# dyollb/segmantic

Measured on AMD Instinct MI355X. Metric: 3D UNet train voxels/s on 128^3 bf16, higher is better.
Workload: dtype bf16

## Files before the change

### include/segmi.h

```cpp
#ifndef SEGMI_H_
#define SEGMI_H_

#include <stddef.h>
#include <stdint.h>

#ifdef __cplusplus
extern "C" {
#endif

#define SEGMI_VERSION 1

enum { SEGMI_F32 = 0, SEGMI_BF16 = 1, SEGMI_F16 = 2 };
enum { SEGMI_OK = 0, SEGMI_EINVAL = -1, SEGMI_EUNSUPPORTED = -2, SEGMI_ELAUNCH = -3,
       SEGMI_EDATA = -4  };

typedef struct segmi_act {
  void* data;
  int32_t n, d, h, w;
  int32_t c;
  int32_t ld;
} segmi_act;

int segmi_version(void);
const char* segmi_last_error(void);
// ... 113 lines not shown
int segmi_bn_eval_affine(int c, const float* gamma, const float* beta,
                         const float* running_mean, const float* running_var, float eps,
                         float* scale, float* shift, void* stream);
int segmi_bn_act_fwd(int dtype, const segmi_act* x, const segmi_act* y, const float* scale,
                     const float* shift, const float* prelu_alpha, const segmi_act* residual,
                     float dropout_p, uint32_t dropout_seed, void* stream);
int segmi_bn_act_bwd_rows(const segmi_act* x);
int segmi_bn_act_bwd_reduce(int dtype, const segmi_act* dy, const segmi_act* x,
                            const float* mean, const float* invstd, const float* gamma,
                            const float* beta, const float* prelu_alpha, float* red_partials,
                            float dropout_p, uint32_t dropout_seed,
                            const segmi_bn_bwd_fin* fin , void* stream);
int segmi_bn_act_bwd_finalize(const float* red_partials, int rows, int c, double count,
                              const float* gamma, const float* invstd, float* dgamma,
                              float* dbeta, float* dalpha, float* coef, void* stream);
int segmi_bn_act_bwd_fused_ok(int dtype, const segmi_act* dy, const segmi_act* x, const segmi_act* dx);
int segmi_bn_act_bwd_fused_rows(const segmi_act* x);
int segmi_bn_act_bwd_fused_wgs(int dtype, const segmi_act* x, int max_wgs);
int segmi_bn_act_bwd_fused(int dtype, const segmi_act* dy, const segmi_act* x, const segmi_act* dx,
                           const float* mean, const float* invstd, const float* gamma, const float* beta,
                           const float* prelu_alpha, float* red_partials, const segmi_bn_bwd_fin* fin,
                           int max_wgs, void* stream);
unsigned segmi_fused_timeouts(int reset);
int segmi_fused_test_hook(unsigned poll_limit, int no_publish);
int segmi_bn_act_bwd_apply(int dtype, const segmi_act* dy, const segmi_act* x,
                           const segmi_act* dx, const float* mean, const float* invstd,
                           const float* gamma, const float* beta, const float* prelu_alpha,
                           const float* coef, float dropout_p, uint32_t dropout_seed, void* stream);
int segmi_bn_act_bwd_apply_conv_ok(int dtype, const segmi_act* dy, const segmi_act* x, const segmi_act* dx,
                                   const segmi_act* out);
int segmi_bn_act_bwd_apply_conv(int dtype, const segmi_act* dy, const segmi_act* x, const segmi_act* dx,
                                const float* mean, const float* invstd, const float* gamma, const float* beta,
                                const float* prelu_alpha, const float* coef, const segmi_act* out,
                                const void* packed, void* stream);

int segmi_add(int dtype, const segmi_act* a, const segmi_act* b, const segmi_act* out,
              void* stream);
int segmi_cast_copy(int src_dtype, const segmi_act* src, int dst_dtype, const segmi_act* dst,
                    void* stream);
int segmi_nchw_to_ndhwc(const float* src, int dst_dtype, const segmi_act* dst, void* stream);
int segmi_ndhwc_to_nchw(int src_dtype, const segmi_act* src, float* dst, void* stream);

int segmi_dice_chunks(const segmi_act* logits);
int segmi_softmax_dice_fwd(int dtype, const segmi_act* logits, const float* labels,
                           float* partials, float* coef, float* loss, float smooth_nr,
                           float smooth_dr, void* stream);
int segmi_softmax_dice_bwd(int dtype, const segmi_act* logits, const float* labels,
                           const float* coef, float grad_scale, const segmi_act* dlogits,
                           float* scratch, float* bias_grad, void* stream);

int segmi_dice_ce_chunks(const segmi_act* logits);
int segmi_softmax_dice_ce_fwd(int dtype, const segmi_act* logits, const float* labels, float* partials,
                              float* coef, float* loss, float smooth_nr, float smooth_dr, float lambda_dice,
                              float lambda_ce, int include_background, const float* class_weight, void* stream);
int segmi_softmax_dice_ce_bwd(int dtype, const segmi_act* logits, const float* labels, const float* coef,
                              float grad_scale, const segmi_act* dlogits, float* scratch, float* bias_grad,
                              void* stream);
int segmi_softmax_dice_ce_bwd_amp(int dtype, const segmi_act* logits, const float* labels, const float* coef,
                                  const float* amp, const segmi_act* dlogits, float* scratch, float* bias_grad,
                                  void* stream);

int segmi_adam_step(float* param, const float* grad, float* exp_avg, float* exp_avg_sq,
                    float* max_exp_avg_sq, int64_t n, double lr, double beta1, double beta2,
                    double eps, double weight_decay, int64_t step, float grad_scale,
                    void* stream);
int segmi_sgd_step(float* param, const float* grad, float* momentum_buf, int64_t n, double lr,
                   double momentum, double weight_decay, int first_step, float grad_scale,
// ... 194 lines not shown
```

### segmantic_amd/_lib.py

```python
from __future__ import annotations

import ctypes as C
import os
from pathlib import Path

import torch

SEGMI_F32 = 0
SEGMI_BF16 = 1
SEGMI_F16 = 2

_LIB_PATH = Path(__file__).resolve().parent / "csrc" / "libsegmi.so"


class Act(C.Structure):

    _fields_ = [("data", C.c_void_p), ("n", C.c_int32), ("d", C.c_int32), ("h", C.c_int32),
                ("w", C.c_int32), ("c", C.c_int32), ("ld", C.c_int32)]


class WpackDesc(C.Structure):

    _fields_ = [("w_src", C.c_void_p), ("scale", C.c_void_p), ("packed", C.c_void_p),
                ("kind", C.c_int32), ("cin_k", C.c_int32), ("cout_k", C.c_int32),
# ... 53 lines not shown
    "segmi_conv3d_fwd_kernel_name": (C.c_char_p, [_i, _AP, _AP, _i, _i]),
    "segmi_conv3d_split_act_ok": (_i, [_i, _AP, _AP, _i, _i]),
    "segmi_conv3d_fwd_split_act": (_i, [_i, _AP, _AP, _P, _P, _P, _i, _i, _i, _P, _P, C.POINTER(BnFin), _P]),
    "segmi_conv3d_fwd": (_i, [_i, _AP, _AP, _P, _P, _i, _P, _P, _AP, _P, _i, _i, C.POINTER(InAffine),
                              C.POINTER(BnBwdSums), C.POINTER(BnFin), _P]),
    "segmi_conv3d_bn_bwd_sums_ok": (_i, [_i, _AP, _AP, _i, _i]),
    "segmi_dectop_ok": (_i, [_i, _AP, _AP]),
    "segmi_dectop_fwd": (_i, [_i, _AP, _AP, _P, _P, _P, _i, _P, _P, _P]),
    "segmi_conv3d_pair_ok": (_i, [_i, _AP, _AP, _AP]),
    "segmi_conv3d_fwd_pair": (_i, [_i, _AP, _AP, _P, _P, _P, _P, _AP, _P, _P, _i, C.POINTER(BnFin),
                                   C.POINTER(Windows), _P]),
    "segmi_convT3d_stats_rows": (_i, [_i, _AP, _AP]),
    "segmi_convT3d_fwd": (_i, [_i, _AP, _AP, _P, _P, _P, _P, _AP, _P, C.POINTER(BnFin), _P]),
    "segmi_conv3d_wgrad_workspace": (_i64, [_i, _AP, _AP, _i, _i, _i]),
    "segmi_conv3d_wgrad": (_i, [_i, _AP, _AP, _P, _P, _i, _i, _P, C.POINTER(InAffine), _i, _P]),
    "segmi_bias_grad": (_i, [_i, _AP, _P, _P, _P]),
    "segmi_bn_stats_rows": (_i, [_AP]),
    "segmi_bn_stats": (_i, [_i, _AP, _P, _P]),
    "segmi_bn_finalize": (_i, [_P, _i, _i, _d, _P, _P, _P, _P, _f, _f, _P, _P, _P, _P, _P]),
    "segmi_bn_eval_affine": (_i, [_i, _P, _P, _P, _P, _f, _P, _P, _P]),
    "segmi_bn_act_fwd": (_i, [_i, _AP, _AP, _P, _P, _P, _AP, _f, C.c_uint32, _P]),
    "segmi_bn_act_bwd_rows": (_i, [_AP]),
    "segmi_bn_act_bwd_reduce": (_i, [_i, _AP, _AP, _P, _P, _P, _P, _P, _P, _f, C.c_uint32,
                                     C.POINTER(BnBwdFin), _P]),
    "segmi_bn_act_bwd_finalize": (_i, [_P, _i, _i, _d, _P, _P, _P, _P, _P, _P, _P]),
    "segmi_bn_act_bwd_fused_ok": (_i, [_i, _AP, _AP, _AP]),
    "segmi_bn_act_bwd_fused_rows": (_i, [_AP]),
    "segmi_bn_act_bwd_fused": (_i, [_i, _AP, _AP, _AP, _P, _P, _P, _P, _P, _P, C.POINTER(BnBwdFin), _i, _P]),
    "segmi_bn_act_bwd_fused_wgs": (_i, [_i, _AP, _i]),
    "segmi_fused_timeouts": (C.c_uint, [_i]),
    "segmi_fused_test_hook": (_i, [C.c_uint, _i]),
    "segmi_bn_act_bwd_apply": (_i, [_i, _AP, _AP, _AP, _P, _P, _P, _P, _P, _P, _f, C.c_uint32, _P]),
    "segmi_bn_act_bwd_apply_conv_ok": (_i, [_i, _AP, _AP, _AP, _AP]),
    "segmi_bn_act_bwd_apply_conv": (_i, [_i, _AP, _AP, _AP, _P, _P, _P, _P, _P, _P, _AP, _P, _P]),
    "segmi_wgrad_cus": (_i, [_i]),
    "segmi_add": (_i, [_i, _AP, _AP, _AP, _P]),
    "segmi_cast_copy": (_i, [_i, _AP, _i, _AP, _P]),
    "segmi_nchw_to_ndhwc": (_i, [_P, _i, _AP, _P]),
    "segmi_ndhwc_to_nchw": (_i, [_i, _AP, _P, _P]),
    "segmi_dice_chunks": (_i, [_AP]),
    "segmi_softmax_dice_fwd": (_i, [_i, _AP, _P, _P, _P, _P, _f, _f, _P]),
    "segmi_softmax_dice_bwd": (_i, [_i, _AP, _P, _P, _f, _AP, _P, _P, _P]),
    "segmi_dice_ce_chunks": (_i, [_AP]),
    "segmi_softmax_dice_ce_fwd": (_i, [_i, _AP, _P, _P, _P, _P, _f, _f, _f, _f, _i, _P, _P]),
    "segmi_softmax_dice_ce_bwd": (_i, [_i, _AP, _P, _P, _f, _AP, _P, _P, _P]),
    "segmi_softmax_dice_ce_bwd_amp": (_i, [_i, _AP, _P, _P, _P, _AP, _P, _P, _P]),
    "segmi_adam_step": (_i, [_P, _P, _P, _P, _P, _i64, _d, _d, _d, _d, _d, _i64, _f, _P]),
    "segmi_sgd_step": (_i, [_P, _P, _P, _i64, _d, _d, _d, _i, _f, _P]),
    "segmi_adabelief_step": (_i, [_P, _P, _P, _P, _i64, _d, _d, _d, _d, _d, _i, _i64, _f, _P]),
    "segmi_softmax_dice_bwd_amp": (_i, [_i, _AP, _P, _P, _P, _AP, _P, _P, _P]),
    "segmi_amp_check_finite": (_i, [_P, _i64, _P, _P]),
    "segmi_amp_update_scale": (_i, [_P, _P, _P, _d, _d, _i, _P]),
    "segmi_adam_step_amp": (_i, [_P, _P, _P, _P, _P, _i64, _d, _d, _d, _d, _d, _P, _P, _f, _P]),
    "segmi_sgd_step_amp": (_i, [_P, _P, _P, _i64, _d, _d, _d, _P, _P, _f, _P]),
    "segmi_adabelief_step_amp": (_i, [_P, _P, _P, _P, _i64, _d, _d, _d, _d, _d, _i, _P, _P, _f, _P]),
    "segmi_sw_gather": (_i, [_i, _AP, _i, _P, _i, _i, _AP, _P]),
    "segmi_sw_scatter_add": (_i, [_i, _AP, _P, _i, _P, _AP, _P, _P]),
    "segmi_sw_finalize": (_i, [_AP, _P, _i, _P, _i, _P]),
    "segmi_sw_blend": (_i, [_i, _P, _i, _i, _P, _i, _P, _i, _P, _i, _i, _i, _i, _i, _i, _P, _i, _i, _i,
                            _P, _i, _P, _P, _i, _i, _P]),
    "segmi_sw_blend_kernel_name": (C.c_char_p, [_i, _P, _i, _i, _P, _i, _P, _i, _P, _i, _i, _i, _i, _P, _i]),
    "segmi_argmax": (_i, [_i, _AP, _P, _i, _P]),
    "segmi_label_counts": (_i, [_P, _P, _i64, _i, _P, _P]),
    "segmi_resample3d": (_i, [_i, _P, _i, _i, _i, _P, _i, _i, _i, _P, _i, _d, _P]),
    "segmi_normalize_workspace": (_i64, [_i, _i64]),
    "segmi_normalize_intensity": (_i, [_P, _i, _i64, _P, _P]),
    "segmi_crop_patches": (_i, [_AP, _P, _P, _P, _i, _i, _AP, _P, _P]),
# ... 95 lines not shown
```

### segmantic_amd/csrc/conv.hip

```cpp
#include "conv_fwd_impl.h"
#include "conv_ring_impl.h"
#include "conv_ks_impl.h"
#include "convt_ps_impl.h"
#include "conv_bnbwd_impl.h"

namespace segmi {

int conv_s2_bnbwd_bf16(const ConvBnBwdParams& p, hipStream_t st);
int conv_s2_bnbwd_f16(const ConvBnBwdParams& p, hipStream_t st);

int conv_mfma_f32(const ConvParams& p, int ksize, int stride, hipStream_t st);
int conv_mfma_bf16(const ConvParams& p, int ksize, int stride, hipStream_t st);
int conv_mfma_f16(const ConvParams& p, int ksize, int stride, hipStream_t st);
int convt_mfma_f32(const ConvTParams& p, hipStream_t st);
int convt_mfma_bf16(const ConvTParams& p, hipStream_t st);
int convt_mfma_f16(const ConvTParams& p, hipStream_t st);
static inline int conv_mfma_dt(int dtype, const ConvParams& p, int ksize, int stride, hipStream_t st) {
  if (dtype == SEGMI_F32) return conv_mfma_f32(p, ksize, stride, st);
  return dtype == SEGMI_F16 ? conv_mfma_f16(p, ksize, stride, st) : conv_mfma_bf16(p, ksize, stride, st);
}
static inline int convt_mfma_dt(int dtype, const ConvTParams& p, hipStream_t st) {
  if (dtype == SEGMI_F32) return convt_mfma_f32(p, st);
  return dtype == SEGMI_F16 ? convt_mfma_f16(p, st) : convt_mfma_bf16(p, st);
}
// ... 246 lines not shown
                              int stride) {
  if (!act_ok(in) || !act_ok(out) || !dtype_h16(dtype) || !mfma_ok(in->c, out->c)) return 0;
  return ksize == 3 && stride == 1 && conv_ring_ok(dtype, in->c, ksize, stride, out) ? 1 : 0;
}

int segmi_conv3d_bn_bwd_sums_ok(int dtype, const segmi_act* in, const segmi_act* out, int ksize,
                                int stride) {
  if (!act_ok(in) || !act_ok(out) || !dtype_h16(dtype)) return 0;
  return ((in->c == 16 && out->c == 16) || (in->c == 32 && out->c == 32)) && ksize == 3 && stride == 1 &&
                 conv_ring_ok(dtype, in->c, ksize, stride, out) ? 1 : 0;
}

int segmi_bn_act_bwd_apply_conv_ok(int dtype, const segmi_act* dy, const segmi_act* x, const segmi_act* dx,
                                   const segmi_act* out) {
  if (!dtype_h16(dtype) || !act_ok(dy) || !act_ok(x) || !act_ok(dx) || !act_ok(out)) return 0;
  const segmi_act* a3[3] = {dy, x, dx};
  for (const segmi_act* a : a3) {
    if (a->n != dy->n || a->d != dy->d || a->h != dy->h || a->w != dy->w || a->c != 16) return 0;
    if (a->ld % 8 != 0 || ((uintptr_t)a->data % 16) != 0) return 0;
  }
  if (out->n != dy->n || out->d != out_extent(dy->d, 3, 2) || out->h != out_extent(dy->h, 3, 2) ||
      out->w != out_extent(dy->w, 3, 2))
    return 0;
  if (!(out->c == 16 || out->c == 32 || out->c == 64) || out->ld % 4 != 0 || ((uintptr_t)out->data % 8) != 0)
    return 0;
  const int64_t vox = (int64_t)dy->d * dy->h * dy->w;
  if (vox * dy->ld * 2 >= (1ll << 31) || vox * x->ld * 2 >= (1ll << 31) || vox * dx->ld * 2 >= (1ll << 31)) return 0;
  return out->w >= 16 ? 1 : 0;
}

int segmi_bn_act_bwd_apply_conv(int dtype, const segmi_act* dy, const segmi_act* x, const segmi_act* dx,
                                const float* mean, const float* invstd, const float* gamma, const float* beta,
                                const float* prelu_alpha, const float* coef, const segmi_act* out,
                                const void* packed, void* stream) {
  SEGMI_CHECK_ARG(segmi_bn_act_bwd_apply_conv_ok(dtype, dy, x, dx, out) && mean && invstd && coef && packed,
                  "bn_act_bwd_apply_conv: not eligible (ask segmi_bn_act_bwd_apply_conv_ok) or bad arguments");
  SEGMI_CHECK_ARG(dx->data != dy->data && dx->data != x->data,
                  "bn_act_bwd_apply_conv: dx must not alias dy or x (halo voxels are re-read by neighbouring tiles)");
  ConvBnBwdParams p{};
  p.dy = dy->data; p.x = x->data; p.dx = dx->data; p.out = out->data; p.wfrag = packed;
  p.mean = mean; p.invstd = invstd; p.gamma = gamma; p.beta = beta; p.alpha = prelu_alpha; p.coef = coef;
  p.N = dy->n; p.Di = dy->d; p.Hi = dy->h; p.Wi = dy->w; p.Do = out->d; p.Ho = out->h; p.Wo = out->w;
  p.Cout = out->c; p.ldy = dy->ld; p.ldx = x->ld; p.lddx = dx->ld; p.ldo = out->ld;
  p.ntiles_total = out->c / 16;
  return dtype == SEGMI_F16 ? conv_s2_bnbwd_f16(p, (hipStream_t)stream) : conv_s2_bnbwd_bf16(p, (hipStream_t)stream);
}

int segmi_conv3d_fwd(int dtype, const segmi_act* in, const segmi_act* out, const void* packed,
                     const float* w_src, int w_kind, const float* bias,
                     const float* prelu_alpha, const segmi_act* residual,
                     float* stats_partials, int ksize, int stride, const segmi_in_affine* in_tf,
                     const segmi_bn_bwd_sums* bn_bwd, const segmi_bn_fin* stats_fin, void* stream) {
  SEGMI_CHECK_ARG(!stats_fin || (stats_partials && bn_fin_ok(stats_fin)),
                  "conv3d: stats_fin needs stats_partials and its output pointers");
  if (bn_bwd && bn_bwd->fin)
    SEGMI_CHECK_ARG(bn_bwd->fin->count > 0 && bn_bwd->fin->coef, "conv3d: bn_bwd->fin needs count and coef");
  if (bn_bwd)
    SEGMI_CHECK_ARG(bn_bwd->x && act_ok(bn_bwd->x) && bn_bwd->mean && bn_bwd->invstd && bn_bwd->partials &&
                        segmi_conv3d_bn_bwd_sums_ok(dtype, in, out, ksize, stride) && !prelu_alpha &&
                        !stats_partials && bn_bwd->x->n == out->n && bn_bwd->x->d == out->d &&
                        bn_bwd->x->h == out->h && bn_bwd->x->w == out->w && bn_bwd->x->c == out->c &&
                        bn_bwd->x->ld % 4 == 0 && ((uintptr_t)bn_bwd->x->data % 8) == 0,
                    "conv3d: this launch cannot take BatchNorm-backward sums (ask segmi_conv3d_bn_bwd_sums_ok)");
  if (in_tf)
    SEGMI_CHECK_ARG(in_tf->scale && in_tf->shift && segmi_conv3d_in_affine_ok(dtype, in, out, ksize, stride),
                    "conv3d: this layer cannot take an input transform (ask segmi_conv3d_in_affine_ok)");
  SEGMI_CHECK_ARG(dtype_ok(dtype), "conv3d: bad dtype %d", dtype);
  SEGMI_CHECK_ARG(act_ok(in) && act_ok(out), "conv3d: bad activation view");
  SEGMI_CHECK_ARG((ksize == 1 || ksize == 3) && (stride == 1 || stride == 2),
                  "conv3d: unsupported ksize/stride %d/%d", ksize, stride);
  SEGMI_CHECK_ARG(!(ksize == 1 && stride != 1), "conv3d: k1 is stride 1 only");
  SEGMI_CHECK_ARG(in->n == out->n && out->d == out_extent(in->d, ksize, stride) &&
                      out->h == out_extent(in->h, ksize, stride) &&
                      out->w == out_extent(in->w, ksize, stride),
                  "conv3d: output extent [%d,%d,%d,%d] does not match input [%d,%d,%d,%d] k%d s%d",
                  out->n, out->d, out->h, out->w, in->n, in->d, in->h, in->w, ksize, stride);
  if (residual)
// ... 141 lines not shown
```

### segmantic_amd/csrc/conv_bnbwd_impl.h

```cpp
#pragma once
#include "conv_fwd_impl.h"

#include <type_traits>
#ifndef SEGMI_BNBWD_KB
#define SEGMI_BNBWD_KB 6
#endif

namespace segmi {

constexpr int kBnBwdLds = 12 * 128 * 32;

struct ConvBnBwdParams {
  const void* dy;
  const void* x;
  void* dx;
  void* out;
  const void* wfrag;
  const float* mean; const float* invstd; const float* gamma; const float* beta; const float* alpha;
  const float* coef;
  int N, Di, Hi, Wi, Do, Ho, Wo, Cout, ldy, ldx, lddx, ldo;
  int tz, ty, tx, ntiles_total;
};

template <typename T, int NT>
__global__ __launch_bounds__(256, 3) void conv_s2_bnbwd_kernel(ConvBnBwdParams p) {
  constexpr int S = 2, KS = 3, TD = 2, TH = 4, TW = 16;
  using G = ConvGeom<T, 16, KS, S, TD, TH, TW>;
  static_assert(G::SPT == 2 && G::ROWB == 32 && G::CPR == 2, "16 bf16 channels per voxel row");
  extern __shared__ __attribute__((aligned(16))) char smem[];
  const int tid = threadIdx.x, lane = tid & 63;
  const int wave = __builtin_amdgcn_readfirstlane(tid >> 6);
  const int g = lane >> 4, r = lane & 15;

  int t = blockIdx.x;
  const int txi = t % p.tx; t /= p.tx;
  const int tyi = t % p.ty; t /= p.ty;
  const int tzi = t % p.tz;
  const int n = t / p.tz;
  const int oz0 = tzi * TD, oy0 = tyi * TH, ox0 = txi * TW;
  const int iz0 = oz0 * S - 1, iy0 = oy0 * S - 1, ix0 = ox0 * S - 1;

  const int half = wave & 1;
  const int c8 = half * 8;
  f32x2 m2[4], i2[4], g2[4], b2[4], c02[4], c12[4], gi2[4];
#pragma unroll
  for (int q = 0; q < 4; ++q)
#pragma unroll
    for (int h = 0; h < 2; ++h) {
      const int ch = c8 + 2 * q + h;
      m2[q][h] = p.mean[ch];
      i2[q][h] = p.invstd[ch];
      g2[q][h] = p.gamma ? p.gamma[ch] : 1.f;
      b2[q][h] = p.beta ? p.beta[ch] : 0.f;
      c02[q][h] = p.coef[ch];
      c12[q][h] = p.coef[16 + ch];
    }
#pragma unroll
  for (int q = 0; q < 4; ++q) {
    gi2[q] = g2[q] * i2[q];
    asm volatile("" : "+v"(gi2[q]), "+v"(b2[q]));
  }
  const bool has_alpha = p.alpha != nullptr;
  const float alpha = has_alpha ? *p.alpha : 1.f;

  constexpr int NVX = G::HD * G::HH * G::HW;
  constexpr int NLD = (NVX + 127) / 128;
  constexpr int KB = SEGMI_BNBWD_KB;
  constexpr int NB = NLD / KB;
  static_assert(NLD % KB == 0 && NLD * 128 * G::ROWB <= kBnBwdLds, "batches cover the tile, LDS covers the batches");
  const int vbase = (wave >> 1) * 64 + lane;
  const int64_t svox = (int64_t)p.Di * p.Hi * p.Wi;
  const __amdgpu_buffer_rsrc_t rs_dy = __builtin_amdgcn_make_buffer_rsrc(
      (void*)((const char*)p.dy + (n * svox * p.ldy + c8) * 2), 0, (int)(svox * p.ldy * 2 - c8 * 2), 0x00020000);
  const __amdgpu_buffer_rsrc_t rs_x = __builtin_amdgcn_make_buffer_rsrc(
      (void*)((const char*)p.x + (n * svox * p.ldx + c8) * 2), 0, (int)(svox * p.ldx * 2 - c8 * 2), 0x00020000);
  const __amdgpu_buffer_rsrc_t rs_dx = __builtin_amdgcn_make_buffer_rsrc(
      (void*)((char*)p.dx + (n * svox * p.lddx + c8) * 2), 0, (int)(svox * p.lddx * 2 - c8 * 2), 0x00020000);
  constexpr int kOob = (int)0x80000000;
  frag_t dzr[2][KB], xr[2][KB];
  int code[2][KB];
  auto issue = [&](int b, frag_t (&dz)[KB], frag_t (&xx)[KB], int (&cd)[KB]) {
#pragma unroll
    for (int k = 0; k < KB; ++k) {
      const int v = vbase + 128 * (b * KB + k);
      const int hx = v % G::HW, hy = (v / G::HW) % G::HH, hz = v / (G::HW * G::HH);
      const int z = iz0 + hz, y = iy0 + hy, x = ix0 + hx;
      const bool inside = (v < NVX) & ((unsigned)z < (unsigned)p.Di) & ((unsigned)y < (unsigned)p.Hi) &
                          ((unsigned)x < (unsigned)p.Wi);
      const int vox = (z * p.Hi + y) * p.Wi + x;
      cd[k] = inside ? 2 * vox + (int)((hz >= 1) & (hy >= 1) & (hx >= 1)) : -1;
      dz[k] = __builtin_amdgcn_raw_buffer_load_b128(rs_dy, inside ? vox * p.ldy * 2 : kOob, 0, 0);
      xx[k] = __builtin_amdgcn_raw_buffer_load_b128(rs_x, inside ? vox * p.ldx * 2 : kOob, 0, 0);
    }
  };
  auto commit = [&](int b, frag_t (&dz)[KB], frag_t (&xx)[KB], int (&cd)[KB], auto ha) {
    constexpr bool HA = decltype(ha)::value;
#pragma unroll
    for (int k = 0; k < KB; ++k) {
      const int v = vbase + 128 * (b * KB + k);
      frag_t val;
#pragma unroll
      for (int q = 0; q < 4; ++q) {
        const f32x2 a{H16<T>::lo(xx[k][q]), H16<T>::hi(xx[k][q])};
        const f32x2 d{H16<T>::lo(dz[k][q]), H16<T>::hi(dz[k][q])};
        const f32x2 o2 = bn_bwd_apply_elem2g<HA>(a, d, m2[q], i2[q], g2[q], b2[q], c02[q], c12[q], gi2[q], alpha);
        val[q] = cd[k] >= 0 ? H16<T>::pack2(o2[0], o2[1]) : 0u;
      }
      __builtin_amdgcn_raw_buffer_store_b128(val, rs_dx, ((cd[k] >= 0) & ((cd[k] & 1) != 0)) ? (cd[k] >> 1) * p.lddx * 2 : kOob, 0, 0);
      *reinterpret_cast<frag_t*>(smem + v * G::ROWB + half * 16) = val;
    }
  };
  auto stage = [&](auto ha) {
    issue(0, dzr[0], xr[0], code[0]);
#pragma unroll
    for (int b = 0; b < NB; ++b) {
      if (b + 1 < NB) issue(b + 1, dzr[(b + 1) & 1], xr[(b + 1) & 1], code[(b + 1) & 1]);
      commit(b, dzr[b & 1], xr[b & 1], code[b & 1], ha);
    }
  };
  if (has_alpha) stage(std::true_type{});
  else stage(std::false_type{});
  constexpr int WD = NT <= 2 ? 4 : 2;
  const char* wb = (const char*)p.wfrag + lane * 16;
  frag_t wq[WD][NT];
#pragma unroll
  for (int s = 0; s < WD; ++s)
#pragma unroll
    for (int j = 0; j < NT; ++j)
      wq[s][j] = *reinterpret_cast<const frag_t*>(wb + ((int64_t)s * p.ntiles_total + j) * 1024);
  __syncthreads();

  f32x4 acc[G::VTW][NT];
#pragma unroll
  for (int i = 0; i < G::VTW; ++i)
#pragma unroll
    for (int j = 0; j < NT; ++j) acc[i][j] = f32x4{0.f, 0.f, 0.f, 0.f};
  int vaddr[G::VTW];
#pragma unroll
  for (int i = 0; i < G::VTW; ++i) {
    const int idx = (wave * G::VTW + i) * 16 + r;
    const int x = idx % TW, y = (idx / TW) % TH, z = idx / (TW * TH);
    vaddr[i] = ((z * S * G::HH + y * S) * G::HW + x * S) * G::ROWB;
  }
#pragma unroll
  for (int s = 0; s < G::NSTEP; ++s) {
    const int t0 = 2 * s, t1 = 2 * s + 1;
    const int o0 = ((t0 / (KS * KS)) * G::HH + (t0 / KS) % KS) * G::HW + t0 % KS;
    const int o1 = t1 < G::NTAPS ? ((t1 / (KS * KS)) * G::HH + (t1 / KS) % KS) * G::HW + t1 % KS : 0;
    const int loff = ((g >> 1) ? o1 : o0) * G::ROWB + (g & 1) * 16;
    frag_t wf[NT];
#pragma unroll
    for (int j = 0; j < NT; ++j) wf[j] = wq[s % WD][j];
    if (s + WD < G::NSTEP) {
#pragma unroll
      for (int j = 0; j < NT; ++j)
        wq[s % WD][j] = *reinterpret_cast<const frag_t*>(wb + ((int64_t)(s + WD) * p.ntiles_total + j) * 1024);
    }
#pragma unroll
    for (int i = 0; i < G::VTW; ++i) {
      const frag_t a = *reinterpret_cast<const frag_t*>(smem + vaddr[i] + loff);
#pragma unroll
      for (int j = 0; j < NT; ++j) acc[i][j] = mma16<T>(wf[j], a, acc[i][j]);
    }
  }

  T* outp = (T*)p.out;
#pragma unroll
  for (int i = 0; i < G::VTW; ++i) {
    const int idx = (wave * G::VTW + i) * 16 + r;
    const int oz = oz0 + idx / (TW * TH), oy = oy0 + (idx / TW) % TH, ox = ox0 + idx % TW;
    if (oz < p.Do && oy < p.Ho && ox < p.Wo) {
      const int64_t vox = (((int64_t)n * p.Do + oz) * p.Ho + oy) * p.Wo + ox;
#pragma unroll
      for (int j = 0; j < NT; ++j) store4<T>(outp + vox * p.ldo + j * 16 + 4 * g, acc[i][j]);
    }
  }
}

template <typename T, int NT>
static int launch_conv_s2_bnbwd(ConvBnBwdParams p, hipStream_t st) {
  using G = ConvGeom<T, 16, 3, 2, 2, 4, 16>;
  p.tz = cdiv(p.Do, 2);
  p.ty = cdiv(p.Ho, 4);
  p.tx = cdiv(p.Wo, 16);
  const int64_t nb = (int64_t)p.N * p.tz * p.ty * p.tx;
  SEGMI_CHECK_ARG(nb < (1ll << 31), "bn_act_bwd_apply_conv: too many tiles");
  static_assert(G::LDS_BYTES <= kBnBwdLds, "halo tile fits");
  hipLaunchKernelGGL((conv_s2_bnbwd_kernel<T, NT>), dim3((unsigned)nb), 256, kBnBwdLds, st, p);
  SEGMI_LAUNCH_CHECK("bn_act_bwd_apply_conv");
  return SEGMI_OK;
}

}
```

### segmantic_amd/ops.py

```python
from __future__ import annotations

import ctypes as C
import math
from typing import Optional, Sequence

import numpy as np
import torch

from . import _lib
from ._lib import SEGMI_BF16, SEGMI_F16, SEGMI_F32, Act, BnBwdFin, BnBwdSums, BnFin, InAffine, Windows, check, lib

_DT = {torch.float32: SEGMI_F32, torch.bfloat16: SEGMI_BF16, torch.float16: SEGMI_F16}


def dtype_code(t: torch.Tensor) -> int:
    try:
        return _DT[t.dtype]
    except KeyError:
        raise TypeError(f"unsupported activation dtype {t.dtype} (float32 / bfloat16 / float16 only)")


def _stream() -> int:
    return torch.cuda.current_stream().cuda_stream

# ... 344 lines not shown
                                     _ptr(invstd), _ptr(gamma), _ptr(beta), _ptr(prelu_alpha), _ptr(partials),
                                     C.byref(bf), int(max_wgs), _stream()), "bn_act_bwd_fused")


def bn_act_bwd_fused_wgs(x, max_wgs: int = 0) -> int:
    a = act(x)
    return int(lib.segmi_bn_act_bwd_fused_wgs(dtype_code(x), C.byref(a), int(max_wgs)))


def fused_timeouts(reset: bool = False) -> int:
    return int(lib.segmi_fused_timeouts(1 if reset else 0))


def check_fused_timeouts(where: str = "") -> None:
    n = fused_timeouts(reset=True)
    if n:
        raise RuntimeError(
            f"{n} workgroup(s) of segmi_bn_act_bwd_fused gave up waiting for their launch's last workgroup"
            f"{' (' + where + ')' if where else ''}: the launch was never fully resident (GPU shared with another "
            "process, or CUs masked).  The gradients of that step are NaN and the weights are poisoned: restart "
            "from the last checkpoint with SEGMI_FUSE_BN_BWD_SMALL=0 (three launches, no grid-wide wait).")


def fused_test_hook(poll_limit: int = 0, no_publish: bool = False) -> None:
    check(lib.segmi_fused_test_hook(int(poll_limit), 1 if no_publish else 0), "fused_test_hook")


def bn_act_bwd_apply_conv_ok(dy, x, dx, out) -> bool:
    ady, ax, adx, ao = act(dy), act(x), act(dx), act(out)
    return bool(lib.segmi_bn_act_bwd_apply_conv_ok(dtype_code(x), C.byref(ady), C.byref(ax), C.byref(adx),
                                                   C.byref(ao)))


def bn_act_bwd_apply_conv(dy, x, dx, mean, invstd, gamma, beta, prelu_alpha, coef, out, packed) -> None:
    ady, ax, adx, ao = act(dy), act(x), act(dx), act(out)
    check(lib.segmi_bn_act_bwd_apply_conv(dtype_code(x), C.byref(ady), C.byref(ax), C.byref(adx), _ptr(mean),
                                          _ptr(invstd), _ptr(gamma), _ptr(beta), _ptr(prelu_alpha), _ptr(coef),
                                          C.byref(ao), _ptr(packed), _stream()), "bn_act_bwd_apply_conv")


def bn_act_bwd_finalize(partials, rows, c, count, gamma, invstd, dgamma, dbeta, dalpha,
                        coef) -> None:
    check(lib.segmi_bn_act_bwd_finalize(_ptr(partials), rows, c, float(count), _ptr(gamma),
                                        _ptr(invstd), _ptr(dgamma), _ptr(dbeta), _ptr(dalpha),
                                        _ptr(coef), _stream()), "bn_act_bwd_finalize")


def bn_act_bwd_apply(dy, x, dx, mean, invstd, gamma, beta, prelu_alpha, coef,
                     dropout=(0.0, 0)) -> None:
    ady, ax, adx = act(dy), act(x), act(dx)
    check(lib.segmi_bn_act_bwd_apply(dtype_code(x), C.byref(ady), C.byref(ax), C.byref(adx),
                                     _ptr(mean), _ptr(invstd), _ptr(gamma), _ptr(beta),
                                     _ptr(prelu_alpha), _ptr(coef), float(dropout[0]),
                                     int(dropout[1]) & 0xFFFFFFFF, _stream()),
          "bn_act_bwd_apply")


def add(a, b, out) -> None:
    aa, ao = act(a), act(out)
    ab = act(b) if b is not None else None
    check(lib.segmi_add(dtype_code(a), C.byref(aa), _ref(ab), C.byref(ao), _stream()), "add")


def cast_copy(src, dst) -> None:
    a, b = act(src), act(dst)
    check(lib.segmi_cast_copy(dtype_code(src), C.byref(a), dtype_code(dst), C.byref(b),
                              _stream()), "cast_copy")


def nchw_to_ndhwc(src: torch.Tensor, dst: torch.Tensor) -> None:
    if src.dtype != torch.float32 or not src.is_contiguous():
# ... 1079 lines not shown
```

Before: 3.638 billion.

## Make fused BN-backward stride-2 conv kernel persistent with precomputed halo offsets

Converts the fused BN-activation-backward plus stride-2 conv kernel into a persistent grid-stride loop over tiles, with the grid capped at occupancy-derived residency (or a caller-supplied cap). Per-lane halo offsets are computed once and reused across tiles. Interior tiles take a branch-free load path, and border tiles use packed-coordinate range checks. Staging changes from double-buffered batches to a rolling prefetch of depth PF. The aim is to cut launch/tail overhead and per-voxel index arithmetic, at the cost of more registers (NLD offset arrays plus deeper prefetch), which may reduce occupancy.

New measurement: 3.616 billion. No clear change (-0.6%).

```diff
diff --git a/include/segmi.h b/include/segmi.h
--- a/include/segmi.h
+++ b/include/segmi.h
@@ -169,7 +169,7 @@
 int segmi_bn_act_bwd_apply_conv(int dtype, const segmi_act* dy, const segmi_act* x, const segmi_act* dx,
                                 const float* mean, const float* invstd, const float* gamma, const float* beta,
                                 const float* prelu_alpha, const float* coef, const segmi_act* out,
-                                const void* packed, void* stream);
+                                const void* packed, void* stream, int grid_cap);
 
 int segmi_add(int dtype, const segmi_act* a, const segmi_act* b, const segmi_act* out,
               void* stream);
diff --git a/segmantic_amd/_lib.py b/segmantic_amd/_lib.py
--- a/segmantic_amd/_lib.py
+++ b/segmantic_amd/_lib.py
@@ -109,7 +109,7 @@
     "segmi_fused_test_hook": (_i, [C.c_uint, _i]),
     "segmi_bn_act_bwd_apply": (_i, [_i, _AP, _AP, _AP, _P, _P, _P, _P, _P, _P, _f, C.c_uint32, _P]),
     "segmi_bn_act_bwd_apply_conv_ok": (_i, [_i, _AP, _AP, _AP, _AP]),
-    "segmi_bn_act_bwd_apply_conv": (_i, [_i, _AP, _AP, _AP, _P, _P, _P, _P, _P, _P, _AP, _P, _P]),
+    "segmi_bn_act_bwd_apply_conv": (_i, [_i, _AP, _AP, _AP, _P, _P, _P, _P, _P, _P, _AP, _P, _P, _i]),
     "segmi_wgrad_cus": (_i, [_i]),
     "segmi_add": (_i, [_i, _AP, _AP, _AP, _P]),
     "segmi_cast_copy": (_i, [_i, _AP, _i, _AP, _P]),
diff --git a/segmantic_amd/csrc/conv.hip b/segmantic_amd/csrc/conv.hip
--- a/segmantic_amd/csrc/conv.hip
+++ b/segmantic_amd/csrc/conv.hip
@@ -302,7 +302,7 @@
 int segmi_bn_act_bwd_apply_conv(int dtype, const segmi_act* dy, const segmi_act* x, const segmi_act* dx,
                                 const float* mean, const float* invstd, const float* gamma, const float* beta,
                                 const float* prelu_alpha, const float* coef, const segmi_act* out,
-                                const void* packed, void* stream) {
+                                const void* packed, void* stream, int grid_cap) {
   SEGMI_CHECK_ARG(segmi_bn_act_bwd_apply_conv_ok(dtype, dy, x, dx, out) && mean && invstd && coef && packed,
                   "bn_act_bwd_apply_conv: not eligible (ask segmi_bn_act_bwd_apply_conv_ok) or bad arguments");
   SEGMI_CHECK_ARG(dx->data != dy->data && dx->data != x->data,
@@ -313,6 +313,7 @@
   p.N = dy->n; p.Di = dy->d; p.Hi = dy->h; p.Wi = dy->w; p.Do = out->d; p.Ho = out->h; p.Wo = out->w;
   p.Cout = out->c; p.ldy = dy->ld; p.ldx = x->ld; p.lddx = dx->ld; p.ldo = out->ld;
   p.ntiles_total = out->c / 16;
+  p.grid_cap = grid_cap;
   return dtype == SEGMI_F16 ? conv_s2_bnbwd_f16(p, (hipStream_t)stream) : conv_s2_bnbwd_bf16(p, (hipStream_t)stream);
 }
 
diff --git a/segmantic_amd/csrc/conv_bnbwd_impl.h b/segmantic_amd/csrc/conv_bnbwd_impl.h
--- a/segmantic_amd/csrc/conv_bnbwd_impl.h
+++ b/segmantic_amd/csrc/conv_bnbwd_impl.h
@@ -1,9 +1,14 @@
 #pragma once
 #include "conv_fwd_impl.h"
 
+#include <map>
+#include <mutex>
 #include <type_traits>
-#ifndef SEGMI_BNBWD_KB
-#define SEGMI_BNBWD_KB 6
+#ifndef SEGMI_BNBWD_PF
+#define SEGMI_BNBWD_PF 8
+#endif
+#ifndef SEGMI_BNBWD_PF_BORDER
+#define SEGMI_BNBWD_PF_BORDER 6
 #endif
 
 namespace segmi {
@@ -20,6 +25,7 @@
   const float* coef;
   int N, Di, Hi, Wi, Do, Ho, Wo, Cout, ldy, ldx, lddx, ldo;
   int tz, ty, tx, ntiles_total;
+  int grid_cap;
 };
 
 template <typename T, int NT>
@@ -32,14 +38,6 @@
   const int wave = __builtin_amdgcn_readfirstlane(tid >> 6);
   const int g = lane >> 4, r = lane & 15;
 
-  int t = blockIdx.x;
-  const int txi = t % p.tx; t /= p.tx;
-  const int tyi = t % p.ty; t /= p.ty;
-  const int tzi = t % p.tz;
-  const int n = t / p.tz;
-  const int oz0 = tzi * TD, oy0 = tyi * TH, ox0 = txi * TW;
-  const int iz0 = oz0 * S - 1, iy0 = oy0 * S - 1, ix0 = ox0 * S - 1;
-
   const int half = wave & 1;
   const int c8 = half * 8;
   f32x2 m2[4], i2[4], g2[4], b2[4], c02[4], c12[4], gi2[4];
@@ -65,116 +63,225 @@
 
   constexpr int NVX = G::HD * G::HH * G::HW;
   constexpr int NLD = (NVX + 127) / 128;
-  constexpr int KB = SEGMI_BNBWD_KB;
-  constexpr int NB = NLD / KB;
-  static_assert(NLD % KB == 0 && NLD * 128 * G::ROWB <= kBnBwdLds, "batches cover the tile, LDS covers the batches");
+  static_assert(NLD * 128 * G::ROWB <= kBnBwdLds, "LDS covers the staging passes");
   const int vbase = (wave >> 1) * 64 + lane;
+  constexpr int kOob = (int)0x80000000;
+  constexpr int kHxSh = 0, kHySh = 8, kHzSh = 16, kVSh = 24;
+  constexpr unsigned kGuard = (1u << 6) | (1u << 12) | (1u << 19) | (1u << 25);
+  constexpr unsigned kOwned = 1u << 31;
+  static_assert(G::HW < 64 && G::HH < 16 && (NLD * 128 - 1) / (G::HW * G::HH) < 8, "halo coordinates fit their fields");
+  int rel_dy[NLD], rel_x[NLD], rel_dx[NLD];
+  auto packed = [&](int v) {
+    const int hx = v % G::HW, hy = (v / G::HW) % G::HH, hz = v / (G::HW * G::HH);
+    const bool valid = v < NVX, owned = (hz >= 1) & (hy >= 1) & (hx >= 1);
+    return ((unsigned)hx << kHxSh) | ((unsigned)hy << kHySh) | ((unsigned)hz << kHzSh) | ((valid ? 1u : 0u) << kVSh) |
+           kGuard | ((valid & owned) ? kOwned : 0u);
+  };
+#pragma unroll
+  for (int j = 0; j < NLD; ++j) {
+    const int v = vbase + 128 * j;
+    const int hx = v % G::HW, hy = (v / G::HW) % G::HH, hz = v / (G::HW * G::HH);
+    const bool valid = v < NVX, owned = (hz >= 1) & (hy >= 1) & (hx >= 1);
+    const unsigned rel = ((unsigned)hz * p.Hi + hy) * p.Wi + hx;
+    rel_dy[j] = valid ? (int)(rel * p.ldy * 2) : kOob;
+    rel_x[j] = valid ? (int)(rel * p.ldx * 2) : kOob;
+    rel_dx[j] = (valid & owned) ? (int)(rel * p.lddx * 2) : kOob;
+    asm volatile("" : "+v"(rel_dy[j]), "+v"(rel_x[j]), "+v"(rel_dx[j]));
+  }
   const int64_t svox = (int64_t)p.Di * p.Hi * p.Wi;
-  const __amdgpu_buffer_rsrc_t rs_dy = __builtin_amdgcn_make_buffer_rsrc(
-      (void*)((const char*)p.dy + (n * svox * p.ldy + c8) * 2), 0, (int)(svox * p.ldy * 2 - c8 * 2), 0x00020000);
-  const __amdgpu_buffer_rsrc_t rs_x = __builtin_amdgcn_make_buffer_rsrc(
-      (void*)((const char*)p.x + (n * svox * p.ldx + c8) * 2), 0, (int)(svox * p.ldx * 2 - c8 * 2), 0x00020000);
-  const __amdgpu_buffer_rsrc_t rs_dx = __builtin_amdgcn_make_buffer_rsrc(
-      (void*)((char*)p.dx + (n * svox * p.lddx + c8) * 2), 0, (int)(svox * p.lddx * 2 - c8 * 2), 0x00020000);
-  constexpr int kOob = (int)0x80000000;
-  frag_t dzr[2][KB], xr[2][KB];
-  int code[2][KB];
-  auto issue = [&](int b, frag_t (&dz)[KB], frag_t (&xx)[KB], int (&cd)[KB]) {
-#pragma unroll
-    for (int k = 0; k < KB; ++k) {
-      const int v = vbase + 128 * (b * KB + k);
-      const int hx = v % G::HW, hy = (v / G::HW) % G::HH, hz = v / (G::HW * G::HH);
-      const int z = iz0 + hz, y = iy0 + hy, x = ix0 + hx;
-      const bool inside = (v < NVX) & ((unsigned)z < (unsigned)p.Di) & ((unsigned)y < (unsigned)p.Hi) &
-                          ((unsigned)x < (unsigned)p.Wi);
-      const int vox = (z * p.Hi + y) * p.Wi + x;
-      cd[k] = inside ? 2 * vox + (int)((hz >= 1) & (hy >= 1) & (hx >= 1)) : -1;
-      dz[k] = __builtin_amdgcn_raw_buffer_load_b128(rs_dy, inside ? vox * p.ldy * 2 : kOob, 0, 0);
-      xx[k] = __builtin_amdgcn_raw_buffer_load_b128(rs_x, inside ? vox * p.ldx * 2 : kOob, 0, 0);
-    }
-  };
-  auto commit = [&](int b, frag_t (&dz)[KB], frag_t (&xx)[KB], int (&cd)[KB], auto ha) {
+  const int64_t sb_dy = svox * p.ldy * 2, sb_x = svox * p.ldx * 2, sb_dx = svox * p.lddx * 2;
+  const char* const base_dy = (const char*)p.dy + c8 * 2;
+  const char* const base_x = (const char*)p.x + c8 * 2;
+  char* const base_dx = (char*)p.dx + c8 * 2;
+  __amdgpu_buffer_rsrc_t rs_dy, rs_x, rs_dx;
+  int iz0, iy0, ix0;
+  int org_dy, org_x, org_dx;
+
+  constexpr int PF_IN = SEGMI_BNBWD_PF < NLD ? SEGMI_BNBWD_PF : NLD;
+  constexpr int PF_BD = SEGMI_BNBWD_PF_BORDER < NLD ? SEGMI_BNBWD_PF_BORDER : NLD;
+  frag_t dzr[NLD], xr[NLD];
+  unsigned ins;
+  int vb;
+  auto issue_in = [&](int j) {
+    dzr[j] = __builtin_amdgcn_raw_buffer_load_b128(rs_dy, rel_dy[j], org_dy, 0);
+    xr[j] = __builtin_amdgcn_raw_buffer_load_b128(rs_x, rel_x[j], org_x, 0);
+  };
+  auto issue_bd = [&](int j, unsigned lo, unsigned him) {
+    const unsigned w = packed(vb + 128 * j);
+    const bool inside = (((w - lo) & (him - w)) & kGuard) == kGuard;
+    ins |= inside ? ((int)w < 0 ? 0x10001u : 1u) << j : 0u;
+    dzr[j] = __builtin_amdgcn_raw_buffer_load_b128(rs_dy, inside ? rel_dy[j] + org_dy : kOob, 0, 0);
+    xr[j] = __builtin_amdgcn_raw_buffer_load_b128(rs_x, inside ? rel_x[j] + org_x : kOob, 0, 0);
+  };
+  auto commit = [&](int j, auto ha, auto interior) {
     constexpr bool HA = decltype(ha)::value;
-#pragma unroll
-    for (int k = 0; k < KB; ++k) {
-      const int v = vbase + 128 * (b * KB + k);
-      frag_t val;
-#pragma unroll
-      for (int q = 0; q < 4; ++q) {
-        const f32x2 a{H16<T>::lo(xx[k][q]), H16<T>::hi(xx[k][q])};
-        const f32x2 d{H16<T>::lo(dz[k][q]), H16<T>::hi(dz[k][q])};
-        const f32x2 o2 = bn_bwd_apply_elem2g<HA>(a, d, m2[q], i2[q], g2[q], b2[q], c02[q], c12[q], gi2[q], alpha);
-        val[q] = cd[k] >= 0 ? H16<T>::pack2(o2[0], o2[1]) : 0u;
+    constexpr bool IN = decltype(interior)::value;
+    const int v = vbase + 128 * j;
+    const bool inside = IN || ((ins >> j) & 1u) != 0;
+    frag_t val;
+#pragma unroll
+    for (int q = 0; q < 4; ++q) {
+      const f32x2 a{H16<T>::lo(xr[j][q]), H16<T>::hi(xr[j][q])};
+      const f32x2 d{H16<T>::lo(dzr[j][q]), H16<T>::hi(dzr[j][q])};
+      const f32x2 o2 = bn_bwd_apply_elem2g<HA>(a, d, m2[q], i2[q], g2[q], b2[q], c02[q], c12[q], gi2[q], alpha);
+      val[q] = inside ? H16<T>::pack2(o2[0], o2[1]) : 0u;
+    }
+    if constexpr (IN) {
+      __builtin_amdgcn_raw_buffer_store_b128(val, rs_dx, rel_dx[j], org_dx, 0);
+    } else {
+      const bool mine = ((ins >> (16 + j)) & 1u) != 0;
+      __builtin_amdgcn_raw_buffer_store_b128(val, rs_dx, mine ? rel_dx[j] + org_dx : kOob, 0, 0);
+    }
+    *reinterpret_cast<frag_t*>(smem + v * G::ROWB + half * 16) = val;
+  };
+  auto stage = [&](auto ha, auto interior) {
+    constexpr bool IN = decltype(interior)::value;
+    unsigned lo = 0, him = 0;
+    if constexpr (!IN) {
+      const int lox = ix0 < 0 ? 1 : 0, loy = iy0 < 0 ? 1 : 0, loz = iz0 < 0 ? 1 : 0;
+      const int hix = min(G::HW, p.Wi - ix0), hiy = min(G::HH, p.Hi - iy0), hiz = min(G::HD, p.Di - iz0);
+      lo = ((unsigned)lox << kHxSh) | ((unsigned)loy << kHySh) | ((unsigned)loz << kHzSh) | (1u << kVSh);
+      him = ((unsigned)(hix - 1) << kHxSh) | ((unsigned)(hiy - 1) << kHySh) | ((unsigned)(hiz - 1) << kHzSh) |
+            (1u << kVSh) | 2u * kGuard;
+      ins = 0;
+      vb = vbase;
+      asm volatile("" : "+v"(vb));
+    }
+    auto issue = [&](int j) {
+      if constexpr (IN) issue_in(j);
+      else issue_bd(j, lo, him);
+    };
+    constexpr int PF = IN ? PF_IN : PF_BD;
+#pragma unroll
+    for (int j = 0; j < PF; ++j) issue(j);
+    __syncthreads();
+#pragma unroll
+    for (int j = 0; j < NLD; ++j) {
+      if (j + PF < NLD) issue(j + PF);
+      commit(j, ha, interior);
+    }
+  };
+
+  constexpr int WD = NT <= 2 ? 4 : 2;
+  T* outp = (T*)p.out;
+
+  int txi, tyi, tzi, n, sx, sy, sz, sn;
+  {
+    int t = blockIdx.x;
+    txi = t % p.tx; t /= p.tx;
+    tyi = t % p.ty; t /= p.ty;
+    tzi = t % p.tz;
+    n = t / p.tz;
+    t = gridDim.x;
+    sx = t % p.tx; t /= p.tx;
+    sy = t % p.ty; t /= p.ty;
+    sz = t % p.tz;
+    sn = t / p.tz;
+  }
+  auto walk = [&](auto ha) {
+  for (; n < p.N;) {
+    const int oz0 = tzi * TD, oy0 = tyi * TH, ox0 = txi * TW;
+    iz0 = oz0 * S - 1, iy0 = oy0 * S - 1, ix0 = ox0 * S - 1;
+    rs_dy = __builtin_amdgcn_make_buffer_rsrc((void*)(base_dy + n * sb_dy), 0, (int)(sb_dy - c8 * 2), 0x00020000);
+    rs_x = __builtin_amdgcn_make_buffer_rsrc((void*)(base_x + n * sb_x), 0, (int)(sb_x - c8 * 2), 0x00020000);
+    rs_dx = __builtin_amdgcn_make_buffer_rsrc((void*)(base_dx + n * sb_dx), 0, (int)(sb_dx - c8 * 2), 0x00020000);
+    const int org = (iz0 * p.Hi + iy0) * p.Wi + ix0;
+    org_dy = org * p.ldy * 2, org_x = org * p.ldx * 2, org_dx = org * p.lddx * 2;
+    const bool interior = (iz0 >= 0) & (iy0 >= 0) & (ix0 >= 0) & (iz0 + G::HD <= p.Di) & (iy0 + G::HH <= p.Hi) &
+                          (ix0 + G::HW <= p.Wi);
+    if (interior) stage(ha, std::true_type{});
+    else stage(ha, std::false_type{});
+    int wlane = lane * 16;
+    asm volatile("" : "+v"(wlane));
+    const char* wb = (const char*)p.wfrag + wlane;
+    frag_t wq[WD][NT];
+#pragma unroll
+    for (int s = 0; s < WD; ++s)
+#pragma unroll
+      for (int j = 0; j < NT; ++j)
+        wq[s][j] = *reinterpret_cast<const frag_t*>(wb + ((int64_t)s * p.ntiles_total + j) * 1024);
+    __syncthreads();
+
+    int gt = g, rt = r;
+    asm volatile("" : "+v"(gt), "+v"(rt));
+    int vaddr[G::VTW];
+#pragma unroll
+    for (int i = 0; i < G::VTW; ++i) {
+      const int idx = (wave * G::VTW + i) * 16 + rt;
+      const int x = idx % TW, y = (idx / TW) % TH, z = idx / (TW * TH);
+      vaddr[i] = ((z * S * G::HH + y * S) * G::HW + x * S) * G::ROWB;
+    }
+    f32x4 acc[G::VTW][NT];
+#pragma unroll
+    for (int i = 0; i < G::VTW; ++i)
+#pragma unroll
+      for (int j = 0; j < NT; ++j) acc[i][j] = f32x4{0.f, 0.f, 0.f, 0.f};
+#pragma unroll
+    for (int s = 0; s < G::NSTEP; ++s) {
+      const int t0 = 2 * s, t1 = 2 * s + 1;
+      const int o0 = ((t0 / (KS * KS)) * G::HH + (t0 / KS) % KS) * G::HW + t0 % KS;
+      const int o1 = t1 < G::NTAPS ? ((t1 / (KS * KS)) * G::HH + (t1 / KS) % KS) * G::HW + t1 % KS : 0;
+      const int loff = ((gt >> 1) ? o1 : o0) * G::ROWB + (gt & 1) * 16;
+      frag_t wf[NT];
+#pragma unroll
+      for (int j = 0; j < NT; ++j) wf[j] = wq[s % WD][j];
+      if (s + WD < G::NSTEP) {
+#pragma unroll
+        for (int j = 0; j < NT; ++j)
+          wq[s % WD][j] = *reinterpret_cast<const frag_t*>(wb + ((int64_t)(s + WD) * p.ntiles_total + j) * 1024);
       }
-      __builtin_amdgcn_raw_buffer_store_b128(val, rs_dx, ((cd[k] >= 0) & ((cd[k] & 1) != 0)) ? (cd[k] >> 1) * p.lddx * 2 : kOob, 0, 0);
-      *reinterpret_cast<frag_t*>(smem + v * G::ROWB + half * 16) = val;
-    }
-  };
-  auto stage = [&](auto ha) {
-    issue(0, dzr[0], xr[0], code[0]);
-#pragma unroll
-    for (int b = 0; b < NB; ++b) {
-      if (b + 1 < NB) issue(b + 1, dzr[(b + 1) & 1], xr[(b + 1) & 1], code[(b + 1) & 1]);
-      commit(b, dzr[b & 1], xr[b & 1], code[b & 1], ha);
-    }
-  };
-  if (has_alpha) stage(std::true_type{});
-  else stage(std::false_type{});
-  constexpr int WD = NT <= 2 ? 4 : 2;
-  const char* wb = (const char*)p.wfrag + lane * 16;
-  frag_t wq[WD][NT];
-#pragma unroll
-  for (int s = 0; s < WD; ++s)
-#pragma unroll
-    for (int j = 0; j < NT; ++j)
-      wq[s][j] = *reinterpret_cast<const frag_t*>(wb + ((int64_t)s * p.ntiles_total + j) * 1024);
-  __syncthreads();
-
-  f32x4 acc[G::VTW][NT];
-#pragma unroll
-  for (int i = 0; i < G::VTW; ++i)
-#pragma unroll
-    for (int j = 0; j < NT; ++j) acc[i][j] = f32x4{0.f, 0.f, 0.f, 0.f};
-  int vaddr[G::VTW];
-#pragma unroll
-  for (int i = 0; i < G::VTW; ++i) {
-    const int idx = (wave * G::VTW + i) * 16 + r;
-    const int x = idx % TW, y = (idx / TW) % TH, z = idx / (TW * TH);
-    vaddr[i] = ((z * S * G::HH + y * S) * G::HW + x * S) * G::ROWB;
+#pragma unroll
+      for (int i = 0; i < G::VTW; ++i) {
+        const frag_t a = *reinterpret_cast<const frag_t*>(smem + vaddr[i] + loff);
+#pragma unroll
+        for (int j = 0; j < NT; ++j) acc[i][j] = mma16<T>(wf[j], a, acc[i][j]);
+      }
+    }
+
+#pragma unroll
+    for (int i = 0; i < G::VTW; ++i) {
+      const int idx = (wave * G::VTW + i) * 16 + rt;
+      const int oz = oz0 + idx / (TW * TH), oy = oy0 + (idx / TW) % TH, ox = ox0 + idx % TW;
+      if (oz < p.Do && oy < p.Ho && ox < p.Wo) {
+        const int64_t vox = (((int64_t)n * p.Do + oz) * p.Ho + oy) * p.Wo + ox;
+#pragma unroll
+        for (int j = 0; j < NT; ++j) store4<T>(outp + vox * p.ldo + j * 16 + 4 * gt, acc[i][j]);
+      }
+    }
+
+    txi += sx;
+    int c = txi >= p.tx ? 1 : 0;
+    txi -= c ? p.tx : 0;
+    tyi += sy + c;
+    c = tyi >= p.ty ? 1 : 0;
+    tyi -= c ? p.ty : 0;
+    tzi += sz + c;
+    c = tzi >= p.tz ? 1 : 0;
+    tzi -= c ? p.tz : 0;
+    n += sn + c;
   }
-#pragma unroll
-  for (int s = 0; s < G::NSTEP; ++s) {
-    const int t0 = 2 * s, t1 = 2 * s + 1;
-    const int o0 = ((t0 / (KS * KS)) * G::HH + (t0 / KS) % KS) * G::HW + t0 % KS;
-    const int o1 = t1 < G::NTAPS ? ((t1 / (KS * KS)) * G::HH + (t1 / KS) % KS) * G::HW + t1 % KS : 0;
-    const int loff = ((g >> 1) ? o1 : o0) * G::ROWB + (g & 1) * 16;
-    frag_t wf[NT];
-#pragma unroll
-    for (int j = 0; j < NT; ++j) wf[j] = wq[s % WD][j];
-    if (s + WD < G::NSTEP) {
-#pragma unroll
-      for (int j = 0; j < NT; ++j)
-        wq[s % WD][j] = *reinterpret_cast<const frag_t*>(wb + ((int64_t)(s + WD) * p.ntiles_total + j) * 1024);
-    }
-#pragma unroll
-    for (int i = 0; i < G::VTW; ++i) {
-      const frag_t a = *reinterpret_cast<const frag_t*>(smem + vaddr[i] + loff);
-#pragma unroll
-      for (int j = 0; j < NT; ++j) acc[i][j] = mma16<T>(wf[j], a, acc[i][j]);
-    }
-  }
-
-  T* outp = (T*)p.out;
-#pragma unroll
-  for (int i = 0; i < G::VTW; ++i) {
-    const int idx = (wave * G::VTW + i) * 16 + r;
-    const int oz = oz0 + idx / (TW * TH), oy = oy0 + (idx / TW) % TH, ox = ox0 + idx % TW;
-    if (oz < p.Do && oy < p.Ho && ox < p.Wo) {
-      const int64_t vox = (((int64_t)n * p.Do + oz) * p.Ho + oy) * p.Wo + ox;
-#pragma unroll
-      for (int j = 0; j < NT; ++j) store4<T>(outp + vox * p.ldo + j * 16 + 4 * g, acc[i][j]);
-    }
-  }
+  };
+  if (has_alpha) walk(std::true_type{});
+  else walk(std::false_type{});
+}
+
+template <typename T, int NT>
+static int conv_s2_bnbwd_capacity() {
+  static std::mutex mu;
+  static std::map<int, int> cache;
+  int dev = 0;
+  if (hipGetDevice(&dev) != hipSuccess) return 0;
+  std::lock_guard<std::mutex> lk(mu);
+  auto it = cache.find(dev);
+  if (it != cache.end()) return it->second;
+  int per_cu = 0, cus = 0;
+  if (hipOccupancyMaxActiveBlocksPerMultiprocessor(&per_cu, reinterpret_cast<const void*>(conv_s2_bnbwd_kernel<T, NT>),
+                                                   256, kBnBwdLds) != hipSuccess)
+    per_cu = 0;
+  if (hipDeviceGetAttribute(&cus, hipDeviceAttributeMultiprocessorCount, dev) != hipSuccess) cus = 0;
+  (void)hipGetLastError();
+  const int64_t cap = (int64_t)per_cu * cus;
+  return cache[dev] = (int)(cap < (1 << 30) ? cap : (1 << 30));
 }
 
 template <typename T, int NT>
@@ -183,9 +290,12 @@
   p.tz = cdiv(p.Do, 2);
   p.ty = cdiv(p.Ho, 4);
   p.tx = cdiv(p.Wo, 16);
-  const int64_t nb = (int64_t)p.N * p.tz * p.ty * p.tx;
+  int64_t nb = (int64_t)p.N * p.tz * p.ty * p.tx;
   SEGMI_CHECK_ARG(nb < (1ll << 31), "bn_act_bwd_apply_conv: too many tiles");
+  SEGMI_CHECK_ARG(p.grid_cap >= 0, "bn_act_bwd_apply_conv: negative grid cap");
   static_assert(G::LDS_BYTES <= kBnBwdLds, "halo tile fits");
+  const int cap = p.grid_cap > 0 ? p.grid_cap : conv_s2_bnbwd_capacity<T, NT>();
+  if (cap > 0 && nb > cap) nb = cap;
   hipLaunchKernelGGL((conv_s2_bnbwd_kernel<T, NT>), dim3((unsigned)nb), 256, kBnBwdLds, st, p);
   SEGMI_LAUNCH_CHECK("bn_act_bwd_apply_conv");
   return SEGMI_OK;
diff --git a/segmantic_amd/ops.py b/segmantic_amd/ops.py
--- a/segmantic_amd/ops.py
+++ b/segmantic_amd/ops.py
@@ -400,11 +400,13 @@
                                                    C.byref(ao)))
 
 
-def bn_act_bwd_apply_conv(dy, x, dx, mean, invstd, gamma, beta, prelu_alpha, coef, out, packed) -> None:
+def bn_act_bwd_apply_conv(dy, x, dx, mean, invstd, gamma, beta, prelu_alpha, coef, out, packed,
+                          grid_cap=None) -> None:
     ady, ax, adx, ao = act(dy), act(x), act(dx), act(out)
     check(lib.segmi_bn_act_bwd_apply_conv(dtype_code(x), C.byref(ady), C.byref(ax), C.byref(adx), _ptr(mean),
                                           _ptr(invstd), _ptr(gamma), _ptr(beta), _ptr(prelu_alpha), _ptr(coef),
-                                          C.byref(ao), _ptr(packed), _stream()), "bn_act_bwd_apply_conv")
+                                          C.byref(ao), _ptr(packed), _stream(), int(grid_cap or 0)),
+          "bn_act_bwd_apply_conv")
 
 
 def bn_act_bwd_finalize(partials, rows, c, count, gamma, invstd, dgamma, dbeta, dalpha,
```
